# profi248/backuwup

Measured on AMD Instinct MI355X. Metric: GB/s chunked+hashed+deduped (whole node, 1/2/4/8 GPU), bit-exact vs CPU, higher is better.
Workload: dtype u8

## Files before the change

backuwup_amd/csrc/bw_blake3.hip:

```cpp
#include "bw_device.h"
#include "bw_internal.h"

namespace bw {
#if BW_CLOCK_STAMPS
__device__ ClockLog* g_clk_b3 = nullptr;
void clock_log_register_b3(void* log) { hipMemcpyToSymbol(HIP_SYMBOL(g_clk_b3), &log, sizeof(log)); }
#endif


typedef uint32_t u32x4_a4 __attribute__((ext_vector_type(4), aligned(4)));

__device__ uint32_t g_b3_dummy[36];

__device__ __forceinline__ void load_words(const uint32_t* src, uint32_t w[17]) {
    const u32x4_a4* q = (const u32x4_a4*)src;
    const u32x4_a4 a = q[0], b = q[1], c = q[2], d = q[3];
    w[0] = a.x; w[1] = a.y; w[2] = a.z; w[3] = a.w; w[4] = b.x; w[5] = b.y; w[6] = b.z; w[7] = b.w;
    w[8] = c.x; w[9] = c.y; w[10] = c.z; w[11] = c.w; w[12] = d.x; w[13] = d.y; w[14] = d.z; w[15] = d.w;
    w[16] = src[16];
}

template <bool PREFETCH>
__device__ __forceinline__ void b3_leaf(const uint8_t* __restrict__ data, uint64_t ls, uint32_t ll, uint64_t bend,
                                        uint64_t t, uint32_t root, uint32_t cv[8]) {
// ... 195 lines not shown
        switch (u + 16) { B3_CUT_CASE8(16) B3_CUT_CASE8(24) B3_CUT_CASE8(32) B3_CUT_CASE8(40) default: break; }
    }
}

__device__ __attribute__((aligned(128))) uint4 g_b3_zero_line[8];

__device__ __forceinline__ void b3_line_load(const uint4* __restrict__ src, uint32_t w[32]) {
#pragma unroll
    for (int k = 0; k < 8; k++) {
        const uint4 v = src[k];
        w[4 * k] = v.x; w[4 * k + 1] = v.y; w[4 * k + 2] = v.z; w[4 * k + 3] = v.w;
    }
}

__device__ __forceinline__ void b3_line_block(uint32_t m[16], uint32_t blk, uint32_t glen, uint32_t nblk, uint64_t n,
                                              uint64_t first, uint32_t cv[8], uint32_t (*s_leaf)[8][256], int me) {
    const uint32_t left = glen - 64 * blk;
    const uint32_t blen = glen == 0 ? 0 : (left < 64 ? left : 64);
    if (blen < 64) {
        const uint32_t whole = blen >> 2, rem = blen & 3;
        const uint32_t pmask = rem ? 0xffffffffu >> (32 - 8 * rem) : 0;
#pragma unroll
        for (uint32_t i = 0; i < 16; i++) m[i] = i < whole ? m[i] : (i == whole ? m[i] & pmask : 0);
    }
    const uint32_t bil = blk & 15, leaf = blk >> 4;
    const bool last = bil == 15 || blk + 1 == nblk;
    if (bil == 0) b3_iv(cv);
    uint32_t flags = bil == 0 ? B3_CHUNK_START : 0;
    if (last) flags |= B3_CHUNK_END | (n == 1 ? B3_ROOT : 0);
    b3_compress(cv, m, blen, first + leaf, flags);
    if (last) {
#pragma unroll
        for (int i = 0; i < 8; i++) s_leaf[leaf][i][me] = cv[i];
    }
}

constexpr uint64_t B3_SMALL_LEAVES = 64;

template <bool COH>
__device__ __forceinline__ uint32_t cv_ld(const uint32_t* p) {
    if constexpr (COH) return __hip_atomic_load(const_cast<uint32_t*>(p), __ATOMIC_RELAXED, __HIP_MEMORY_SCOPE_AGENT);
    else return *p;
}
template <bool COH>
__device__ __forceinline__ void cv_st(uint32_t* p, uint32_t v) {
    if constexpr (COH) __hip_atomic_store(p, v, __ATOMIC_RELAXED, __HIP_MEMORY_SCOPE_AGENT);
    else *p = v;
}
__device__ __forceinline__ void wave_mem_drain() { asm volatile("s_waitcnt vmcnt(0)" ::: "memory"); }

template <bool COH>
__device__ __forceinline__ void b3_small_blob(uint64_t blob, const uint64_t* ctr, const BlobArrays& b,
                                              uint32_t* __restrict__ cv_buf, uint8_t* __restrict__ digests);
template <bool COH, int NT = 64>
__device__ __forceinline__ void b3_upper_wave(uint64_t blob, uint64_t len, const BlobArrays& b, uint32_t* __restrict__ cv_buf,
                              uint32_t* __restrict__ cv_tmp, uint8_t* __restrict__ digests);

template <int MINW, bool FUSED>
__global__ __launch_bounds__(256, MINW) void k_b3_lines(const uint8_t* __restrict__ data, const uint64_t* ctr,
                                                        BlobArrays b, uint32_t* __restrict__ cv_buf,
                                                        uint32_t* __restrict__ cv_tmp, uint8_t* __restrict__ digests) {
    const uint64_t ng = ctr[C_NGROUPS];
    const uint64_t g0 = (uint64_t)blockIdx.x * blockDim.x + threadIdx.x;
    const bool live = g0 < ng;
    if (FUSED ? (ng == 0 || g0 - (threadIdx.x & 63) >= ng) : !live) return;
#if BW_CLOCK_STAMPS
    ClockStamp clk((blockIdx.x & 3) == 0 ? g_clk_b3 : nullptr, 1);
#endif
    const uint64_t g = live ? g0 : ng - 1;
    const uint64_t nb = ctr[C_NBLOBS];
    uint64_t lo = 0, hi = nb;
    while (lo < hi) {
        const uint64_t mid = (lo + hi) >> 1;
        if (b.goff[mid] <= g) lo = mid + 1;
        else hi = mid;
    }
    const uint64_t blob = lo - 1;
    BW_ASSERT(lo >= 1 && blob < b.cap);
    const uint64_t start = b.start[blob], len = b.len[blob], gi = g - b.goff[blob];
    const uint32_t gs = b.gshift, G = 1u << gs;
    BW_ASSERT(gs <= 2 && start + len <= b.data_len && (gi << gs) * B3_LEAF_BYTES <= (len ? len - 1 : 0));
    const uint64_t n = len == 0 ? 1 : (len + B3_LEAF_BYTES - 1) / B3_LEAF_BYTES;
    const uint64_t first = gi << gs;
    const uint32_t k = (uint32_t)(n - first < G ? n - first : G);
    __shared__ uint32_t s_leaf[4][8][256];
    const int me = threadIdx.x;
    const uint8_t* gp = data + start + first * B3_LEAF_BYTES;
    const uint32_t o = (uint32_t)((uintptr_t)gp & 127);
    const uint32_t q = o >> 2, sh = o & 3;
    const uint32_t uq = __builtin_amdgcn_readfirstlane(q);
    uint32_t cv[8];
    if (__builtin_amdgcn_ballot_w64(q != uq) == 0) {
        const uint64_t rest = len - first * B3_LEAF_BYTES;
        const uint32_t glen = len == 0 ? 0 : (uint32_t)(rest < G * B3_LEAF_BYTES ? rest : G * B3_LEAF_BYTES);
        const uint32_t nblk = glen == 0 ? 1 : (glen + 63) / 64;
        const uint4* lp = (const uint4*)(gp - o);
        const uint32_t nlines = glen == 0 ? 0 : (o + glen + 127) / 128;
        uint32_t a[32], c[32];
        b3_line_load(nlines > 0 ? lp : g_b3_zero_line, a);
        b3_line_load(nlines > 1 ? lp + 8 : g_b3_zero_line, c);
#pragma unroll 1
        for (uint32_t p = 0;; p += 2) {
            uint32_t m[16];
            b3_cut<0>(a, c, uq, sh, m);
            b3_line_block(m, 2 * p, glen, nblk, n, first, cv, s_leaf, me);
            if (2 * p + 1 >= nblk) break;
            b3_cut<1>(a, c, uq, sh, m);
            b3_line_load(p + 2 < nlines ? lp + 8 * (p + 2) : g_b3_zero_line, a);
            b3_line_block(m, 2 * p + 1, glen, nblk, n, first, cv, s_leaf, me);
// ... 16 lines not shown
            for (int i = 0; i < 8; i++) s_leaf[t][i][me] = cv[i];
        }
    }
    uint32_t acc[8], r[8];
#pragma unroll
    for (int i = 0; i < 8; i++) acc[i] = s_leaf[0][i][me];
    if (k >= 2) {
#pragma unroll
        for (int i = 0; i < 8; i++) r[i] = s_leaf[1][i][me];
        b3_parent(acc, r, (n == 2 || (n == 4 && false)) ? B3_ROOT : 0, acc);
    }
    if (k == 4) {
        uint32_t l2[8], l3[8];
#pragma unroll
        for (int i = 0; i < 8; i++) { l2[i] = s_leaf[2][i][me]; l3[i] = s_leaf[3][i][me]; }
        b3_parent(l2, l3, 0, r);
        b3_parent(acc, r, n == 4 ? B3_ROOT : 0, acc);
    } else if (k == 3) {
#pragma unroll
        for (int i = 0; i < 8; i++) r[i] = s_leaf[2][i][me];
        b3_parent(acc, r, n == 3 ? B3_ROOT : 0, acc);
    }
    if (n <= G) store_digest(digests + blob * 32, acc);
    else {
        uint32_t* o8 = cv_buf + g * 8;
#pragma unroll
        for (int i = 0; i < 8; i++) cv_st<FUSED>(o8 + i, acc[i]);
    }
    if constexpr (FUSED) {
        const uint32_t lane = threadIdx.x & 63;
        const bool upper = live && n > G;
        const uint64_t pb = bw_shfl_up64(blob, 1);
        const bool head = upper && (lane == 0 || pb != blob);
        const uint64_t H = __ballot(head), U = __ballot(upper);
        if (H == 0) return;
        wave_mem_drain();
        bool complete = false;
        if (head) {
            const uint64_t above = H & ~((2ull << lane) - 1);
            const uint32_t end = above ? (uint32_t)__builtin_ctzll(above) : 64u;
            const uint64_t run = (end == 64 ? ~0ull : ((1ull << end) - 1)) & ~((1ull << lane) - 1);
            const uint32_t cnt = (uint32_t)__popcll(U & run);
            const uint32_t total = (uint32_t)((n + G - 1) >> gs);
            const uint32_t old = __hip_atomic_fetch_add(b.gdone + blob, cnt, __ATOMIC_RELAXED, __HIP_MEMORY_SCOPE_AGENT);
            BW_ASSERT(old + cnt <= total);
            complete = old + cnt == total;
            if (complete) b.gdone[blob] = 0;
        }
        const uint64_t C = __ballot(complete);
        if (C == 0) return;
        for (uint64_t m = C; m; m &= m - 1) {
            const int h = __builtin_ctzll(m);
            const uint64_t cb = bw_shfl64(blob, h), cl = bw_shfl64(len, h);
            if (cl > (uint64_t)B3_SMALL_LEAVES * B3_LEAF_BYTES) b3_upper_wave<true>(cb, cl, b, cv_buf, cv_tmp, digests);
        }
        if (complete) b3_small_blob<true>(blob, ctr, b, cv_buf, digests);
    }
}


template <bool COH>
__device__ __forceinline__ void b3_small_blob(uint64_t blob, const uint64_t* ctr, const BlobArrays& b,
                                              uint32_t* __restrict__ cv_buf, uint8_t* __restrict__ digests) {
    if (blob >= ctr[C_NBLOBS]) return;
    const uint64_t len = b.len[blob];
    const uint64_t n = len == 0 ? 1 : (len + B3_LEAF_BYTES - 1) / B3_LEAF_BYTES;
    const uint32_t gs = b.gshift;
    if (n <= (1u << gs) || n > B3_SMALL_LEAVES) return;
    uint32_t* g = cv_buf + b.goff[blob] * 8;
    const uint32_t m2 = (uint32_t)(n >> gs);
    const bool tail = (n & ((1u << gs) - 1)) != 0;
    uint32_t depth = 0;
    for (uint32_t i = 0; i < m2; i++) {
        uint32_t carry[8];
#pragma unroll
        for (int w = 0; w < 8; w++) carry[w] = cv_ld<COH>(g + i * 8 + w);
        for (uint32_t c = i + 1; (c & 1) == 0; c >>= 1) {
            uint32_t l[8];
            depth--;
#pragma unroll
            for (int w = 0; w < 8; w++) l[w] = cv_ld<COH>(g + depth * 8 + w);
            b3_parent(l, carry, (!tail && i + 1 == m2 && depth == 0) ? B3_ROOT : 0, carry);
        }
#pragma unroll
        for (int w = 0; w < 8; w++) cv_st<COH>(g + depth * 8 + w, carry[w]);
        depth++;
    }
    uint32_t acc[8];
    bool have = false;
    if (tail) {
#pragma unroll
        for (int w = 0; w < 8; w++) acc[w] = cv_ld<COH>(g + m2 * 8 + w);
        have = true;
    }
    while (depth > 0) {
        depth--;
        uint32_t t[8];
#pragma unroll
        for (int w = 0; w < 8; w++) t[w] = cv_ld<COH>(g + depth * 8 + w);
        if (!have) {
#pragma unroll
            for (int w = 0; w < 8; w++) acc[w] = t[w];
            have = true;
        } else {
            b3_parent(t, acc, depth == 0 ? B3_ROOT : 0, acc);
        }
    }
    store_digest(digests + blob * 32, acc);
}

__device__ __forceinline__ void b3_shfl8(const uint32_t x[8], int src, uint32_t out[8]) {
#pragma unroll
    for (int w = 0; w < 8; w++) out[w] = __shfl(x[w], src, 64);
}

template <bool COH, int NT>
__device__ __forceinline__ void b3_upper_wave(uint64_t blob, uint64_t len, const BlobArrays& b, uint32_t* __restrict__ cv_buf,
                              uint32_t* __restrict__ cv_tmp, uint8_t* __restrict__ digests) {
    static_assert(NT == 64 || NT == 256, "a wave or a 4-wave workgroup per blob");
    const uint32_t lane = threadIdx.x & 63, t = threadIdx.x & (NT - 1);
    const uint64_t n = (len + B3_LEAF_BYTES - 1) / B3_LEAF_BYTES;
    uint32_t* src = cv_buf + b.goff[blob] * 8;
    uint32_t* dst = cv_tmp + b.goff[blob] * 8;
    const uint32_t gs = b.gshift;
    uint64_t cnt = n >> gs;
    bool have = (n & ((1u << gs) - 1)) != 0;
    uint32_t acc[8];
#pragma unroll
    for (int w = 0; w < 8; w++) acc[w] = 0;
    if (have && t == NT - 1) {
#pragma unroll
        for (int w = 0; w < 8; w++) acc[w] = cv_ld<COH>(src + cnt * 8 + w);
    }
    int l = (int)gs;
    while (cnt > 64) {
        const bool spine = cnt & 1;
        const uint64_t next = cnt / 2;
        for (uint64_t base = 0; base < next; base += NT - 1) {
            const uint64_t i = base + t;
            const bool pair = t < NT - 1 && i < next;
            const bool fold = t == NT - 1 && base == 0 && spine && have;
            if (pair || fold) {
                uint32_t L[8], R[8], P[8];
                const uint64_t li = pair ? 2 * i : cnt - 1;
#pragma unroll
                for (int w = 0; w < 8; w++) L[w] = cv_ld<COH>(src + li * 8 + w);
#pragma unroll
                for (int w = 0; w < 8; w++) R[w] = pair ? cv_ld<COH>(src + (li + 1) * 8 + w) : acc[w];
                b3_parent(L, R, 0, P);
                if (pair) {
#pragma unroll
                    for (int w = 0; w < 8; w++) cv_st<COH>(dst + i * 8 + w, P[w]);
                } else {
#pragma unroll
                    for (int w = 0; w < 8; w++) acc[w] = P[w];
                }
            }
        }
        if (spine && !have && t == NT - 1) {
#pragma unroll
            for (int w = 0; w < 8; w++) acc[w] = cv_ld<COH>(src + (cnt - 1) * 8 + w);
        }
        have |= spine;
        if constexpr (COH) wave_mem_drain();
        if constexpr (NT == 64) {
            __builtin_amdgcn_fence(__ATOMIC_RELEASE, "workgroup");
            __builtin_amdgcn_wave_barrier();
            __builtin_amdgcn_fence(__ATOMIC_ACQUIRE, "workgroup");
        } else {
            __syncthreads();
        }
        uint32_t* t = src;
        src = dst;
        dst = t;
        cnt = next;
        l++;
    }
    if (NT > 64 && t / 64 != (NT - 1) / 64) return;
    uint32_t x[8];
#pragma unroll
    for (int w = 0; w < 8; w++) x[w] = lane < cnt ? cv_ld<COH>(src + lane * 8 + w) : 0;
    for (;;) {
        const bool spine = cnt & 1;
        const uint32_t next = (uint32_t)(cnt / 2);
        uint32_t L[8], R[8], T[8], P[8];
        b3_shfl8(x, (int)(2 * lane) & 63, L);
        b3_shfl8(x, (int)(2 * lane + 1) & 63, R);
        b3_shfl8(x, (int)(cnt - 1), T);
        const bool pair = lane < next;
        const bool fold = lane == 63 && spine && have;
        if (pair || fold) {
            const uint32_t root = pair ? (n == (2ull << l) ? B3_ROOT : 0) : ((n >> (l + 1)) == 0 ? B3_ROOT : 0);
            uint32_t A[8], B[8];
#pragma unroll
            for (int w = 0; w < 8; w++) { A[w] = pair ? L[w] : T[w]; B[w] = pair ? R[w] : acc[w]; }
            b3_parent(A, B, root, P);
        }
        if (lane == 63 && spine) {
#pragma unroll
            for (int w = 0; w < 8; w++) acc[w] = have ? P[w] : T[w];
        }
        have |= spine;
        if (next == 0) break;
        if (pair) {
#pragma unroll
            for (int w = 0; w < 8; w++) x[w] = P[w];
        }
        cnt = next;
        l++;
    }
    if (lane == 63) store_digest(digests + blob * 32, acc);
}

__global__ __launch_bounds__(256) void k_b3_upper(const uint64_t* ctr, BlobArrays b, uint32_t* __restrict__ cv_buf,
                                                  uint32_t* __restrict__ cv_tmp, uint8_t* __restrict__ digests,
                                                  uint32_t small_blocks, uint32_t per_block) {
    if (blockIdx.x < small_blocks) {
        b3_small_blob<false>((uint64_t)blockIdx.x * blockDim.x + threadIdx.x, ctr, b, cv_buf, digests);
        return;
    }
    const uint64_t nblobs = ctr[C_NBLOBS];
    if (per_block) {
        const uint64_t one_group = (uint64_t)B3_LEAF_BYTES << b.gshift;
        for (uint64_t blob = blockIdx.x - small_blocks; blob < nblobs; blob += gridDim.x - small_blocks) {
            const uint64_t len = b.len[blob];
            if (len <= one_group) continue;
            b3_upper_wave<false, 256>(blob, len, b, cv_buf, cv_tmp, digests);
        }
        return;
    }
    const uint64_t waves = (uint64_t)(gridDim.x - small_blocks) * (blockDim.x / 64);
    for (uint64_t blob = (uint64_t)(blockIdx.x - small_blocks) * (blockDim.x / 64) + threadIdx.x / 64; blob < nblobs;
         blob += waves) {
        const uint64_t len = b.len[blob];
        if (len <= (uint64_t)B3_SMALL_LEAVES * B3_LEAF_BYTES) continue;
        b3_upper_wave<false, 64>(blob, len, b, cv_buf, cv_tmp, digests);
    }
}

#ifndef BW_B3_LINES_MINW
#define BW_B3_LINES_MINW 3
#endif
#ifndef B3_UPPER_BLOCK_BLOBS
#define B3_UPPER_BLOCK_BLOBS 8192
#endif

__global__ __launch_bounds__(256, BW_B3_LINES_MINW) void k_b3_calib(uint32_t blocks_per_lane, uint32_t* sink,
                                                                    uint64_t* stamps) {
    uint32_t cv[8], m[16];
    b3_iv(cv);
#pragma unroll
    for (int i = 0; i < 16; i++) m[i] = threadIdx.x * 16 + i + blockIdx.x;
    uint64_t t0 = 0, r0 = 0;
    if (threadIdx.x == 0) {
        t0 = __builtin_amdgcn_s_memtime();
        r0 = __builtin_amdgcn_s_memrealtime();
    }
    for (uint32_t k = 0; k < blocks_per_lane; k++) {
        m[0] ^= k;
        b3_compress(cv, m, 64, k, 0);
    }
    if (threadIdx.x == 0) {
        stamps[2 * blockIdx.x] = __builtin_amdgcn_s_memtime() - t0;
        stamps[2 * blockIdx.x + 1] = __builtin_amdgcn_s_memrealtime() - r0;
    }
    if (cv[0] == 0x9e3779b9u && cv[1] == 0x7f4a7c15u) sink[0] = cv[2];
}

void launch_b3_calib(hipStream_t st, uint32_t n_blocks, uint32_t blocks_per_lane, uint32_t* sink, uint64_t* stamps) {
    hipLaunchKernelGGL(k_b3_calib, dim3(n_blocks), dim3(256), 0, st, blocks_per_lane, sink, stamps);
}

uint32_t b3_calib_blocks_per_cu() { return BW_B3_LINES_MINW; }

void launch_blake3(hipStream_t st, const uint8_t* data, const uint64_t* ctr, BlobArrays b, uint64_t max_blobs,
                   uint64_t max_groups, uint32_t* cv_buf, uint32_t* cv_tmp, uint8_t* digests, int max_leaves,
                   hipEvent_t between, int loads, hipStream_t upper, hipEvent_t leaf_done, hipEvent_t mark) {
    if (!max_blobs) {
        if (leaf_done) hipEventRecord(leaf_done, st);
        return;
    }
#ifndef BW_B3_DYN_LDS
#define BW_B3_DYN_LDS 0
#endif
#if BW_DIAG
    const bool fused = loads == B3_LOADS_LINES && b.gdone;
    if (fused)
        hipLaunchKernelGGL((k_b3_lines<BW_B3_LINES_MINW, true>), dim3((unsigned)((max_groups + 255) / 256)), dim3(256), 0, st,
                           data, ctr, b, cv_buf, cv_tmp, digests);
    else if (loads == B3_LOADS_PAIRS)
        hipLaunchKernelGGL((k_b3_groups<false, 1, true>), dim3((unsigned)((max_groups + 255) / 256)), dim3(256), BW_B3_DYN_LDS, st,
                           data, ctr, b, cv_buf, digests);
    else if (loads == B3_LOADS_PREFETCH)
        hipLaunchKernelGGL((k_b3_groups<true, 1, false>), dim3((unsigned)((max_groups + 255) / 256)), dim3(256), 0, st,
                           data, ctr, b, cv_buf, digests);
    else
#else
    const bool fused = false;
    (void)loads;
#endif
        hipLaunchKernelGGL((k_b3_lines<BW_B3_LINES_MINW, false>), dim3((unsigned)((max_groups + 255) / 256)), dim3(256), 0, st,
                           data, ctr, b, cv_buf, cv_tmp, digests);
    if (leaf_done) hipEventRecord(leaf_done, st);
    if (mark) hipEventRecord(mark, st);
    if (between) hipEventRecord(between, st);
    if (upper != st) hipStreamWaitEvent(upper, between, 0);
    st = upper;
    if (max_leaves > (1 << b.gshift) && !fused) {
        const bool per_block = max_blobs <= B3_UPPER_BLOCK_BLOBS;
        const uint64_t small = per_block ? 0 : (max_blobs + 255) / 256;
        uint64_t big = per_block ? max_blobs : (max_leaves > (int)B3_SMALL_LEAVES ? (max_blobs + 3) / 4 : 0);
        if (big > 4096) big = 4096;
        hipLaunchKernelGGL(k_b3_upper, dim3((unsigned)(small + big)), dim3(256), 0, st, ctr, b, cv_buf, cv_tmp, digests,
                           (uint32_t)small, (uint32_t)per_block);
    }
}

}
```

backuwup_amd/csrc/bw_capi.hip:

```cpp
#include <math.h>
#include <stdio.h>
#include <stdlib.h>
#include <string.h>

#include <algorithm>
#include <atomic>
#include <chrono>
#include <functional>
#include <mutex>
#include <string>
#include <thread>
#include <unordered_map>
#include <vector>

#include "../../include/backuwup_gpu.h"
#include "bw_device.h"
#include "bw_internal.h"
#include "bw_tables.inc"

using namespace bw;

static const uint64_t H_MASKS[26] = BW_MASKS_INIT;

#include "bw_ctx.h"
// ... 450 lines not shown
            return BW_OK;
        case BW_OPT_SPLIT:
            if (v < 1 || v > 2) return BW_EINVAL;
            c->split = (int)v;
            return BW_OK;
        case BW_OPT_SCAN_SMALL_BYTES:
            c->scan_small_bytes = v;
            return c->helper ? bw_set_option(c->helper, opt, v) : BW_OK;
        case BW_OPT_ORDER_HASH:
            if (v > 1) return BW_EINVAL;
            c->order_hash = v != 0;
            return BW_OK;
        case BW_OPT_CAND_CAP:
            c->cand_cap_forced = v;
            return c->helper ? bw_set_option(c->helper, opt, v) : BW_OK;
        case BW_OPT_SCAN_WAVES:
            if (v != 8 && v != 16) return BW_EINVAL;
            c->scan_waves = (int)v;
            return c->helper ? bw_set_option(c->helper, opt, v) : BW_OK;
        case BW_OPT_LATENCY_STREAM:
            if (v && !c->hi) {
                hipSetDevice(c->device);
                int least = 0, greatest = 0;
                HIPCHK(c, hipDeviceGetStreamPriorityRange(&least, &greatest));
                HIPCHK(c, hipStreamCreateWithPriority(&c->hi, hipStreamNonBlocking, greatest));
                for (hipEvent_t* e : {&c->e_scan, &c->e_lat, &c->e_b3, &c->e_end})
                    HIPCHK(c, hipEventCreateWithFlags(e, EV_ORDER));
            }
            c->lat_split = v != 0;
            return BW_OK;
        case BW_OPT_ZSTD_SLOTS:
            if (v < 1 || v > (1u << 20)) return BW_EINVAL;
            hipSetDevice(c->device);
            hipStreamSynchronize(c->stream);
            zstd_work_limits(c->zw, v, 0);
            return BW_OK;
        case BW_OPT_ZSTD_BATCH_BYTES:
            if (v < (1u << 20)) return BW_EINVAL;
            zstd_work_limits(c->zw, 0, v);
            return BW_OK;
        case BW_OPT_B3_LOADS:
            if (v > B3_LOADS_LINES) return BW_EINVAL;
            c->b3_loads = (int)v;
            return c->helper ? bw_set_option(c->helper, opt, v) : BW_OK;
        case BW_OPT_PROFILE_MASK:
            if (__builtin_popcountll(v) < 2 || v >= (2u << BW_N_STAGES)) return BW_EINVAL;
            c->prof_mask = (uint32_t)v;
            return c->helper ? bw_set_option(c->helper, opt, v) : BW_OK;
        case BW_OPT_B3_GROUP:
            if (v != 0 && v != 1 && v != 2 && v != 4) return BW_EINVAL;
            c->b3_group = (int)v;
            return c->helper ? bw_set_option(c->helper, opt, v) : BW_OK;
        case BW_OPT_B3_UPPER:
            if (v > 1) return BW_EINVAL;
            c->b3_fused = v == 1;
            return c->helper ? bw_set_option(c->helper, opt, v) : BW_OK;
        case BW_OPT_SCAN_FIRST:
            if (v > 2) return BW_EINVAL;
            c->scan_first = (int)v;
            return c->helper ? bw_set_option(c->helper, opt, v) : BW_OK;
        case BW_OPT_STAGE_CHUNK:
            if (v < 4096) return BW_EINVAL;
            hipSetDevice(c->device);
            if (c->copy) hipStreamSynchronize(c->copy);
            for (int r = 0; r < STAGE_RING; r++) free_host(c->ring[r]);
            c->stage_chunk = v;
            return BW_OK;
        default: return BW_EINVAL;
    }
}


extern "C" int bw_index_create(int device, bw_index** out) {
    if (!out) return BW_EINVAL;
    *out = nullptr;
    bw_index* x = new bw_index();
    if (int rc = index_init(x, device)) {
        index_release(x);
        return rc;
    }
    *out = x;
    return BW_OK;
}

extern "C" void bw_index_destroy(bw_index* x) { index_release(x); }

extern "C" int bw_attach_index(bw_ctx* c, bw_index* x) {
    if (!c) return BW_EINVAL;
    if (!x) x = c->own_idx;
    if (x->device != c->device) {
        c->err = "index and context live on different devices";
        return BW_EINVAL;
    }
    if (x == c->idx) return BW_OK;
    hipSetDevice(c->device);
    HIPCHK(c, hipStreamSynchronize(c->stream));
    bw_index* old = c->idx;
    if (x != c->own_idx) x->refs++;
    c->idx = x;
    c->idx_mark = 0;
    if (old != c->own_idx) index_release(old);
    if (c->helper) return bw_attach_index(c->helper, x);
    return BW_OK;
}

extern "C" int bw_index_reset(bw_ctx* c, uint64_t hint) {
    if (!c) return BW_EINVAL;
    hipSetDevice(c->device);
// ... 329 lines not shown
        if (int r6 = enqueue_scan()) return r6;
    uint64_t* ctr = slot_ctr(s);
    hipStream_t st = c->stream;

    BlobArrays b{P<uint64_t>(c->b_start), P<uint64_t>(c->b_len), P<uint64_t>(c->b_goff), P<uint32_t>(c->b_file),
                 P<uint32_t>(c->b_kind), P<uint64_t>(c->b_fend), P<uint64_t>(c->b_ghash), max_blobs, data_len,
                 c->b3_fused ? P<uint32_t>(c->b_gdone) : nullptr, gshift};

    const bool split = c->lat_split;
    hipStream_t lat = split ? c->hi : st;
    if (split) {
        HIPCHK(c, hipEventRecord(c->e_scan, st));
        HIPCHK(c, hipStreamWaitEvent(lat, c->e_scan, 0));
    }
    prof_mark(c, BW_STAGE_COMPACT, lat);
    if (ncf)
        launch_compact(lat, d_data, data_len, n_tiles, mk, P<uint32_t>(c->tile_count), P<uint64_t>(c->tile_slots),
                       P<uint64_t>(c->tile_off), P<uint64_t>(c->cand), cand_cap, P<uint32_t>(c->ovf), ctr,
                       P<uint64_t>(c->tile_btot));
    prof_mark(c, BW_STAGE_RESOLVE, lat);
    if (ncf) {
        launch_chains(lat, d_data, data_len, mk, P<uint64_t>(c->cand), P<uint64_t>(c->tile_off), ctr, d_segs,
                      nseg, P<uint64_t>(c->chains), P<uint32_t>(c->chain_n), P<uint64_t>(c->chain_cptr),
                      P<uint64_t>(c->merge), force_serial);
        launch_resolve(lat, d_data, data_len, mk, P<uint64_t>(c->cand), P<uint64_t>(c->tile_off), ctr,
                       d_segs, nseg, d_cfs, ncf, P<uint64_t>(c->chains),
                       P<uint32_t>(c->chain_n), P<uint64_t>(c->merge), P<uint64_t>(c->seg_M), P<uint32_t>(c->seg_cnt),
                       P<uint32_t>(c->cf_invalid), P<uint64_t>(c->fb_starts), P<uint64_t>(c->fb_count), force_serial);
    }
    prof_mark(c, BW_STAGE_ASSEMBLE, lat);
    launch_assemble(lat, ctr, d_units, nunits, d_segs, d_cfs,
                    P<uint64_t>(c->chains), P<uint32_t>(c->chain_n), P<uint64_t>(c->seg_M), P<uint32_t>(c->cf_invalid),
                    P<uint64_t>(c->fb_starts), P<uint64_t>(c->fb_count), b, P<uint64_t>(c->ucnt),
                    P<uint64_t>(c->ubtot));
    if (ncf) launch_cut_hash(lat, d_data, mk, ctr, b, max_blobs);
    else HIPCHK(c, hipMemsetAsync(c->b_ghash.p, 0, max_blobs * 8, lat));
    if (split) {
        HIPCHK(c, hipEventRecord(c->e_lat, lat));
        HIPCHK(c, hipStreamWaitEvent(st, c->e_lat, 0));
    }

    prof_mark(c, BW_STAGE_B3LEAF, st);
    if (do_hash) {
        hipEvent_t mark = c->prof && ((c->prof_mask >> BW_STAGE_B3TREE) & 1) ? c->ev[c->ev_set][BW_STAGE_B3TREE] : nullptr;
        hipEvent_t between = split ? c->e_b3 : nullptr;
        bw_index* x = c->idx;
        std::unique_lock<std::mutex> lk(x->mu, std::defer_lock);
        const bool order = c->order_hash || order_force;
        if (order) {
            lk.lock();
            if (x->hash_tail_set) HIPCHK(c, hipStreamWaitEvent(st, x->hash_tail, 0));
        }
        launch_blake3(st, d_data, ctr, b, max_blobs, max_groups, P<uint32_t>(c->cv), P<uint32_t>(c->cv2),
                      P<uint8_t>(s.digests), max_leaves, between, c->b3_loads, lat, order ? x->hash_tail : nullptr, mark);
        if (order) x->hash_tail_set = true;
    } else {
        prof_mark(c, BW_STAGE_B3TREE, st);
        if (split) {
            HIPCHK(c, hipEventRecord(c->e_b3, st));
            HIPCHK(c, hipStreamWaitEvent(lat, c->e_b3, 0));
        }
        HIPCHK(c, hipMemsetAsync(s.digests.p, 0, max_blobs * 32, lat));
    }
    if (d_data == P<uint8_t>(s.input)) HIPCHK(c, hipEventRecord(s.input_free, st));
    phase(3);
    prof_mark(c, BW_STAGE_DEDUP, lat);
    uint64_t want = 0;
    bool zero_copy = false;
    if (stage)
        if (int r5 = stage_prepare(c, s, max_blobs, &want, &zero_copy)) return r5;
    auto pack = [&](hipStream_t ps) {
        prof_mark(c, BW_STAGE_PACK, ps);
        launch_pack(ps, ctr, b, d_fstart, P<uint8_t>(s.digests), do_dedup ? P<uint8_t>(s.is_dup) : nullptr,
                    slot_records(s), max_blobs, do_dedup ? P<uint64_t>(c->idx->dstate) : nullptr,
                    zero_copy ? (uint8_t*)s.res.p : nullptr, want);
    };
    if (do_dedup) {
        if (int r4 = dedup_device(c, P<uint8_t>(s.digests), ctr + C_DEDUPN, 0, max_blobs, P<uint8_t>(s.is_dup), lat,
                                  pack))
            return r4;
        s.mark = c->idx_mark;
    } else {
        pack(lat);
    }
    phase(4);
    if (split) {
        prof_mark(c, BW_N_STAGES, lat);
        HIPCHK(c, hipEventRecord(c->e_end, lat));
        HIPCHK(c, hipStreamWaitEvent(st, c->e_end, 0));
    }
    if (!split) prof_mark(c, BW_N_STAGES);
    if (c->prof) c->ev_pending[c->ev_set] = true;
    HIPCHK(c, hipGetLastError());
    s.max_blobs = max_blobs;
    s.geo_tiles = n_tiles;
    s.geo_cfiles = ncf;
    s.geo_segs = nseg;
    s.geo_tile_bytes = tile_bytes;
    s.geo_seg_bytes = L;
    s.dedup = do_dedup;
    s.hashed = do_hash;
    s.comm = nullptr;
    s.ex_state = 0;
    s.ex_rc = 0;
    s.ex_first = 0;
    s.ex_n = ~0ull;
    if (stage)
        if (int r5 = stage_results(c, s, zero_copy, want)) return r5;
    phase(5);
    c->host_batches += c->host_timing;
    return BW_OK;
}

static Slot& claim_slot(bw_ctx* c, uint64_t* ticket) {
    const uint64_t t = c->next_ticket++;
    Slot& s = c->slots[(t - 1) % (uint64_t)c->depth];
    if (s.ex_state == 1 && s.comm) exchange_progress(s.comm, &s);
    if (s.ex_state == 2) hipStreamWaitEvent(c->stream, s.done, 0);
    s.ticket = t;
    c->last_ticket = t;
    if (ticket) *ticket = t;
    return s;
}

static const bw_params* params_or_default(const bw_params* prm, bw_params* def) {
    if (prm) return prm;
    bw_params_default(def);
    return def;
}

static int ensure_helper(bw_ctx* c) {
    if (c->helper) return BW_OK;
    bw_ctx* h = nullptr;
    if (int rc = bw_create(c->device, &h)) return rc;
    h->is_helper = true;
    h->depth = c->depth;
    h->scan_small_bytes = c->scan_small_bytes;
    h->cand_cap_forced = c->cand_cap_forced;
    h->b3_loads = c->b3_loads;
    h->scan_waves = c->scan_waves;
    h->b3_group = c->b3_group;
    h->b3_fused = c->b3_fused;
    h->prof_mask = c->prof_mask;
    h->scan_first = c->scan_first;
    if (c->lat_split && bw_set_option(h, BW_OPT_LATENCY_STREAM, 1) != BW_OK) {
        bw_destroy(h);
        return BW_EHIP;
    }
    if (int rc = bw_attach_index(h, c->idx)) {
        bw_destroy(h);
        return rc;
    }
    if (c->prof) bw_profile_enable(h, 1);
    if (!c->e_split) HIPCHK(c, hipEventCreateWithFlags(&c->e_split, EV_ORDER));
    if (!c->e_tail) HIPCHK(c, hipEventCreateWithFlags(&c->e_tail, EV_ORDER));
    c->helper = h;
    return BW_OK;
}

static uint64_t split_point(bw_ctx* c, uint64_t data_len, const uint64_t* flen, uint64_t nf, const bw_params* prm) {
    if (c->split < 2 || c->is_helper || nf < 2 || (prm->flags & (BW_F_NO_DEDUP | BW_F_NO_HASH))) return 0;
    if (data_len > c->split_max) return 0;
    uint64_t total = 0;
    for (uint64_t f = 0; f < nf; f++) total += flen[f];
    if (total < c->split_min) return 0;
    uint64_t acc = 0;
    for (uint64_t f = 0; f + 1 < nf; f++) {
        acc += flen[f];
        if (2 * acc >= total) return f + 1;
    }
    return nf - 1;
}

static int submit_split(bw_ctx* c, Slot& s, const uint8_t* d_data, uint64_t data_len, const uint64_t* foff,
                        const uint64_t* flen, uint64_t nf, const bw_params* prm) {
    s.tail_ticket = 0;
    Masks mk;
    if (int rc = validate_batch(c, data_len, foff, flen, nf, prm, &mk)) return rc;
    const uint64_t f0 = split_point(c, data_len, flen, nf, prm);
    if (!f0) return submit(c, s, d_data, data_len, foff, flen, nf, prm);
    if (int rc = ensure_helper(c)) return rc;
    bw_ctx* h = c->helper;
    HIPCHK(c, hipEventRecord(c->e_split, c->stream));
    if (int rc = submit(c, s, d_data, data_len, foff, flen, f0, prm, true, true)) return rc;
    HIPCHK(c, hipStreamWaitEvent(h->stream, c->e_split, 0));
    uint64_t t2 = 0;
    Slot& s2 = claim_slot(h, &t2);
    if (int rc = submit(h, s2, d_data, data_len, foff + f0, flen + f0, nf - f0, prm, true, true)) {
        s2.ticket = 0;
        c->err = "tail part: " + h->err;
        return rc;
    }
    HIPCHK(c, hipEventRecord(c->e_tail, h->stream));
    HIPCHK(c, hipStreamWaitEvent(c->stream, c->e_tail, 0));
    if (d_data == P<uint8_t>(s.input)) HIPCHK(c, hipEventRecord(s.input_free, c->stream));
// ... 737 lines not shown
```

backuwup_amd/csrc/bw_ctx.h:

```cpp
#pragma once
#include <atomic>
#include <functional>
#include <mutex>
#include <string>
#include <thread>
#include <vector>

#include "../../include/backuwup_gpu.h"
#include "bw_internal.h"

using namespace bw;

namespace bwx {

struct DevBuf {
    void* p = nullptr;
    size_t cap = 0;
};

struct PinBuf {
    void* p = nullptr;
    size_t cap = 0;
};

// ... 32 lines not shown

using namespace bwx;

struct bw_index {
    int device = 0;
    std::mutex mu;
    std::atomic<int> refs{1};
    DevBuf table, log, dstate;
    uint64_t table_cap = 0, log_cap = 0;
    uint64_t log_hi = 0;
    uint64_t enq_total = 0;
    hipEvent_t tail = nullptr;
    bool tail_set = false;
    hipStream_t tail_stream = nullptr;
    hipEvent_t hash_tail = nullptr, scan_tail = nullptr;
    bool hash_tail_set = false, scan_tail_set = false;
};

struct bw_ctx {
    int device = 0;
    hipStream_t own = nullptr, stream = nullptr, copy = nullptr;
    std::string err;

    DevBuf tile_count, tile_slots, tile_off, tile_btot, cand, ovf;
    DevBuf meta, chains, chain_n, chain_cptr, merge, seg_M, seg_cnt, cf_invalid, fb_starts, fb_count;
    DevBuf b_start, b_len, b_goff, b_file, b_kind, b_fend, b_ghash;
    DevBuf b_gdone;
    DevBuf cv, cv2, data, scratch, ucnt, ubtot;
    DevBuf bk_blk, bk_pack, bk_v;
    DevBuf ex_rbk, ex_v, ex_rv;
    hipStream_t ex_st = nullptr;

    Slot slots[MAX_DEPTH];
    int depth = 2;
    uint64_t next_ticket = 1, last_ticket = 0;
    uint64_t last_n = 0;
    int split = 1;
    uint64_t split_min = 64ull << 20, split_max = 4ull << 30;
    bw_ctx* helper = nullptr;
    bool is_helper = false;
    hipEvent_t e_split = nullptr, e_tail = nullptr;
    Slot sync_slot;

    PinBuf ring[STAGE_RING];
    hipEvent_t ring_ev[STAGE_RING] = {};
    bool ring_set[STAGE_RING] = {};
    uint64_t stage_chunk = 64ull << 20;

    uint64_t scan_small_bytes = SCAN_SMALL_BYTES;
    bool order_hash = false;
    uint64_t cand_cap_forced = 0;
    int b3_group = 0;
    bool b3_fused = false;
    int b3_loads = B3_LOADS_LINES;
    int scan_waves = 16;
    bool lat_split = false;
    hipStream_t hi = nullptr;
    hipEvent_t e_scan = nullptr, e_lat = nullptr, e_b3 = nullptr, e_end = nullptr;
    uint64_t cand_override = 0;

    DevBuf seal_items, seal_keys, seal_parts, seal_ok, seal_io;
    PinBuf seal_stage;
    hipEvent_t seal_done = nullptr;
    bool seal_pending = false;

    DevBuf pk_blobs, pk_files, pk_hdr, pk_src, pk_out, ix_io, ix_tab, ix_dig;
    std::vector<PackBlob> h_pk_blobs;
    std::vector<PackFileDesc> h_pk_files;
    hipEvent_t pk_done = nullptr;
    bool pk_pending = false;

    PinBuf msg_stage;

    ZstdWork* zw = nullptr;
    struct ZsLane {
        hipStream_t st = nullptr;
        hipStream_t own_st = nullptr;
        hipEvent_t ready = nullptr;
        ZstdWork* w = nullptr;
        std::thread th;
        uint64_t ticket = 0;
        std::vector<uint64_t> so, sl, dof, fl;
        int rc = 0;
        std::string err;
    };
    ZsLane zs_lanes[BW_ZSTD_LANES];
    uint64_t zs_next = 1;
    DevBuf zs_io;
    DevBuf pk_stage;
    std::vector<uint64_t> pk_stage_off, pk_stage_len;

    bw_index* own_idx = nullptr;
    bw_index* idx = nullptr;
    uint64_t idx_mark = 0;

    bool host_timing = false;
    double host_ms[6] = {};
    uint64_t host_batches = 0;

    bool prof = false;
    uint32_t prof_mask = (2u << BW_N_STAGES) - 1;
    int scan_first = 2;
    hipEvent_t ev[2][BW_N_STAGES + 1] = {};
    bool ev_pending[2] = {false, false};
    int ev_set = 0;
    double stage_ms[BW_N_STAGES] = {};
// ... 35 lines not shown
```

backuwup_amd/csrc/bw_internal.h:

```cpp
#pragma once
#include <algorithm>
#include <string>
#include <thread>
#include <vector>
#include <hip/hip_runtime.h>
#include <stdint.h>

#include "../../include/backuwup_gpu.h"

#ifndef BW_DIAG
#define BW_DIAG 0
#endif

namespace bw {

constexpr int SCAN_BLOCK = 1024;
#ifndef BW_SCAN_STRIP
#define BW_SCAN_STRIP 2048
#endif
#ifndef BW_SCAN_CAP
#define BW_SCAN_CAP 16
#endif
constexpr int SCAN_STRIP = BW_SCAN_STRIP;
constexpr uint64_t SCAN_TILE = 64ull * SCAN_STRIP;
// ... 55 lines not shown
    uint32_t seg;
    uint32_t cfile;
};

struct BlobArrays {
    uint64_t* start;
    uint64_t* len;
    uint64_t* goff;
    uint32_t* file;
    uint32_t* kind;
    uint64_t* fend;
    uint64_t* ghash;
    uint64_t cap;
    uint64_t data_len;
    uint32_t* gdone = nullptr;
    uint32_t gshift = 2;
};

bool launch_scan(hipStream_t st, const uint8_t* data, uint64_t n_bytes, uint64_t n_tiles,
                 const Masks& mk, uint32_t* tile_count, uint64_t* tile_slots, uint32_t* ovf_list,
                 uint64_t* ctr, int waves );
void launch_compact(hipStream_t st, const uint8_t* data, uint64_t n_bytes, uint64_t n_tiles,
                    const Masks& mk, uint32_t* tile_count, uint64_t* tile_slots,
                    uint64_t* tile_off, uint64_t* cand, uint64_t cand_cap, uint32_t* ovf_list,
                    uint64_t* ctr, uint64_t* scratch );
void launch_chains(hipStream_t st, const uint8_t* data, uint64_t data_len, const Masks& mk, const uint64_t* cand,
                   const uint64_t* tile_off, uint64_t* ctr, const SegDesc* segs, uint64_t nseg,
                   uint64_t* chains, uint32_t* chain_n, uint64_t* chain_cptr, uint64_t* merge,
                   int force_serial);
void launch_resolve(hipStream_t st, const uint8_t* data, uint64_t data_len, const Masks& mk, const uint64_t* cand,
                    const uint64_t* tile_off, uint64_t* ctr, const SegDesc* segs, uint64_t nseg,
                    const CFileDesc* cfiles, uint64_t ncf, const uint64_t* chains,
                    const uint32_t* chain_n, const uint64_t* merge, uint64_t* seg_M,
                    uint32_t* seg_cnt, uint32_t* cf_invalid, uint64_t* fb_starts,
                    uint64_t* fb_count, int force_serial);
void launch_assemble(hipStream_t st, uint64_t* ctr, const UnitDesc* units, uint64_t nunits,
                     const SegDesc* segs, const CFileDesc* cfiles, const uint64_t* chains,
                     const uint32_t* chain_n, const uint64_t* seg_M, const uint32_t* cf_invalid,
                     const uint64_t* fb_starts, const uint64_t* fb_count, BlobArrays b,
                     uint64_t* ucnt , uint64_t* ubtot );
void launch_upload(hipStream_t st, const void* host_src, void* dst, uint64_t bytes);
void launch_zero(hipStream_t st, uint64_t* p, uint32_t n);
void launch_cut_hash(hipStream_t st, const uint8_t* data, const Masks& mk, const uint64_t* ctr,
                     BlobArrays b, uint64_t max_blobs);


enum { B3_LOADS_PREFETCH = 0, B3_LOADS_PAIRS = 1, B3_LOADS_LINES = 2 };
void launch_blake3(hipStream_t st, const uint8_t* data, const uint64_t* ctr, BlobArrays b,
                   uint64_t max_blobs, uint64_t max_groups, uint32_t* cv_buf,
                   uint32_t* cv_tmp , uint8_t* digests, int max_leaves,
                   hipEvent_t between , int loads,
                   hipStream_t upper ,
                   hipEvent_t leaf_done = nullptr ,
                   hipEvent_t mark = nullptr );
void launch_b3_calib(hipStream_t st, uint32_t n_blocks, uint32_t blocks_per_lane, uint32_t* sink, uint64_t* stamps);
uint32_t b3_calib_blocks_per_cu();
enum DState : int { D_LOGLEN = 0, D_NUNIQUE = 1, D_LOST = 2, D_BUCKET_OVF = 3, D_DONE = 4, D_COUNT = 5 };
void launch_table_clear(hipStream_t st, uint64_t* table, uint64_t cap);
void launch_dedup(hipStream_t st, uint64_t* table, uint64_t cap, uint8_t* log, uint64_t* dstate,
                  const uint8_t* digests, const uint64_t* n_dev, uint64_t n_host, uint64_t max_n,
                  uint8_t* is_dup);
void launch_rehash(hipStream_t st, uint64_t* table, uint64_t cap, const uint8_t* log,
                   const uint64_t* dstate, uint64_t max_n);
void launch_partition(hipStream_t st, const uint8_t* digests, uint64_t n, uint32_t n_owners,
                      uint8_t* out, uint64_t* perm, uint64_t* counts_dev);
void launch_scatter(hipStream_t st, const uint8_t* verdict, const uint64_t* perm, uint64_t n,
                    uint8_t* is_dup);
void launch_bucket_partition(hipStream_t st, const uint8_t* digests, const uint64_t* n_dev, uint64_t max_n,
                             uint32_t n_owners, uint64_t cap, uint8_t* out, uint64_t* perm, uint64_t* counts,
                             uint64_t* blk, uint64_t* err);
void launch_bucket_gather(hipStream_t st, const uint8_t* buckets, const uint64_t* counts, uint32_t n_src, uint64_t cap,
                          uint8_t* out, uint64_t* n_out);
void launch_bucket_expand(hipStream_t st, const uint64_t* counts, uint32_t n_src, uint64_t cap, const uint8_t* v_in,
                          uint8_t* v_out);
void launch_bucket_scatter(hipStream_t st, const uint8_t* verdict, const uint64_t* perm, const uint64_t* counts,
                           uint32_t n_owners, uint64_t cap, uint8_t* is_dup, uint8_t* packed = nullptr);
void launch_pack(hipStream_t st, uint64_t* ctr, BlobArrays b, const uint64_t* file_start,
                 const uint8_t* digests, const uint8_t* is_dup, uint8_t* out, uint64_t max_blobs,
                 const uint64_t* dstate, uint8_t* host = nullptr, uint64_t host_n = 0);
void launch_index_snapshot(hipStream_t st, const uint64_t* dstate, uint64_t* ctr);
void launch_owner_partition(hipStream_t st, const uint8_t* digests, const uint64_t* n_dev, uint64_t max_n,
                            uint32_t n_owners, uint8_t* out, uint64_t* perm, uint64_t* msg, uint64_t* blk);
void launch_copy_u64(hipStream_t st, const uint64_t* src, uint64_t* dst, uint32_t n);
void launch_owner_scatter(hipStream_t st, const uint8_t* verdict, const uint64_t* perm, uint64_t n, uint8_t* is_dup,
                          uint8_t* packed);

constexpr uint32_t PIECE_BLOCKS = 8192;
constexpr int SEAL_THREADS = 1024;

struct SealItem {
    uint64_t src_off, len, dst_off, piece0;
    uint32_t nonce[3];
    uint32_t info_len;
    uint8_t info[56];
    uint32_t raw_len, wd;
};

struct SealKey {
    uint32_t rk[60];
    uint32_t H[4], E0[4], HP[4], H64[4];
    uint32_t P[6][4];
    uint32_t R1[4];
};

struct SealPads {
    uint32_t istate[8], ostate[8];
};
// ... 77 lines not shown
```

Baseline: 1942.

## Process multiple upper BLAKE3 trees per wave using sub-wave teams

The upper-tree BLAKE3 kernel now assigns a team of 32 lanes (configurable to 16 or 64) per blob instead of a full wave, so each wave reduces several blobs' chaining-value trees at once. Shuffles are made team-relative, and loops use wave-wide ballots so teams with different depths stay converged. Non-coherent CV loads and stores are also vectorised to 16-byte accesses. This aims to cut idle lanes when most blobs have few groups, at the cost of more divergence and extra iterations for teams with shallow trees.

```diff
diff --git a/backuwup_amd/csrc/bw_blake3.hip b/backuwup_amd/csrc/bw_blake3.hip
--- a/backuwup_amd/csrc/bw_blake3.hip
+++ b/backuwup_amd/csrc/bw_blake3.hip
@@ -271,9 +271,30 @@
 template <bool COH>
 __device__ __forceinline__ void b3_small_blob(uint64_t blob, const uint64_t* ctr, const BlobArrays& b,
                                               uint32_t* __restrict__ cv_buf, uint8_t* __restrict__ digests);
+template <bool COH>
+__device__ __forceinline__ void cv_ld8(const uint32_t* p, uint32_t out[8]) {
+    if constexpr (COH) {
+#pragma unroll
+        for (int w = 0; w < 8; w++) out[w] = cv_ld<true>(p + w);
+    } else {
+        const uint4 a = ((const uint4*)p)[0], c = ((const uint4*)p)[1];
+        out[0] = a.x; out[1] = a.y; out[2] = a.z; out[3] = a.w; out[4] = c.x; out[5] = c.y; out[6] = c.z; out[7] = c.w;
+    }
+}
+template <bool COH>
+__device__ __forceinline__ void cv_st8(uint32_t* p, const uint32_t v[8]) {
+    if constexpr (COH) {
+#pragma unroll
+        for (int w = 0; w < 8; w++) cv_st<true>(p + w, v[w]);
+    } else {
+        ((uint4*)p)[0] = make_uint4(v[0], v[1], v[2], v[3]);
+        ((uint4*)p)[1] = make_uint4(v[4], v[5], v[6], v[7]);
+    }
+}
+
 template <bool COH, int NT = 64>
-__device__ __forceinline__ void b3_upper_wave(uint64_t blob, uint64_t len, const BlobArrays& b, uint32_t* __restrict__ cv_buf,
-                              uint32_t* __restrict__ cv_tmp, uint8_t* __restrict__ digests);
+__device__ __forceinline__ void b3_upper_wave(uint64_t blob, uint64_t len, bool live, const BlobArrays& b,
+                              uint32_t* __restrict__ cv_buf, uint32_t* __restrict__ cv_tmp, uint8_t* __restrict__ digests);
 
 template <int MINW, bool FUSED>
 __global__ __launch_bounds__(256, MINW) void k_b3_lines(const uint8_t* __restrict__ data, const uint64_t* ctr,
@@ -396,7 +417,7 @@
         for (uint64_t m = C; m; m &= m - 1) {
             const int h = __builtin_ctzll(m);
             const uint64_t cb = bw_shfl64(blob, h), cl = bw_shfl64(len, h);
-            if (cl > (uint64_t)B3_SMALL_LEAVES * B3_LEAF_BYTES) b3_upper_wave<true>(cb, cl, b, cv_buf, cv_tmp, digests);
+            if (cl > (uint64_t)B3_SMALL_LEAVES * B3_LEAF_BYTES) b3_upper_wave<true>(cb, cl, true, b, cv_buf, cv_tmp, digests);
         }
         if (complete) b3_small_blob<true>(blob, ctr, b, cv_buf, digests);
     }
@@ -458,81 +479,91 @@
     for (int w = 0; w < 8; w++) out[w] = __shfl(x[w], src, 64);
 }
 
+template <int NT>
+__device__ __forceinline__ bool b3_any(bool p) {
+    if constexpr (NT < 64) return __builtin_amdgcn_ballot_w64(p) != 0;
+    else return p;
+}
+
 template <bool COH, int NT>
-__device__ __forceinline__ void b3_upper_wave(uint64_t blob, uint64_t len, const BlobArrays& b, uint32_t* __restrict__ cv_buf,
-                              uint32_t* __restrict__ cv_tmp, uint8_t* __restrict__ digests) {
-    static_assert(NT == 64 || NT == 256, "a wave or a 4-wave workgroup per blob");
+__device__ __forceinline__ void b3_upper_wave(uint64_t blob, uint64_t len, bool live, const BlobArrays& b,
+                              uint32_t* __restrict__ cv_buf, uint32_t* __restrict__ cv_tmp, uint8_t* __restrict__ digests) {
+    static_assert(NT == 16 || NT == 32 || NT == 64 || NT == 256, "a team, a wave or a 4-wave workgroup per blob");
+    constexpr uint32_t RL = NT < 64 ? NT : 64;
     const uint32_t lane = threadIdx.x & 63, t = threadIdx.x & (NT - 1);
+    const uint32_t rl = lane & (RL - 1), tb = lane & ~(RL - 1);
     const uint64_t n = (len + B3_LEAF_BYTES - 1) / B3_LEAF_BYTES;
-    uint32_t* src = cv_buf + b.goff[blob] * 8;
-    uint32_t* dst = cv_tmp + b.goff[blob] * 8;
+    const uint64_t goff = live ? b.goff[blob] : 0;
+    uint32_t* src = cv_buf + goff * 8;
+    uint32_t* dst = cv_tmp + goff * 8;
     const uint32_t gs = b.gshift;
-    uint64_t cnt = n >> gs;
-    bool have = (n & ((1u << gs) - 1)) != 0;
+    uint64_t cnt = live ? n >> gs : 0;
+    bool have = live && (n & ((1u << gs) - 1)) != 0;
     uint32_t acc[8];
 #pragma unroll
     for (int w = 0; w < 8; w++) acc[w] = 0;
-    if (have && t == NT - 1) {
-#pragma unroll
-        for (int w = 0; w < 8; w++) acc[w] = cv_ld<COH>(src + cnt * 8 + w);
-    }
+    if (have && t == NT - 1) cv_ld8<COH>(src + cnt * 8, acc);
     int l = (int)gs;
-    while (cnt > 64) {
-        const bool spine = cnt & 1;
+    while (b3_any<NT>(cnt > RL)) {
+        const bool act = cnt > RL;
+        const bool spine = act && (cnt & 1);
         const uint64_t next = cnt / 2;
-        for (uint64_t base = 0; base < next; base += NT - 1) {
+        for (uint64_t base = 0; b3_any<NT>(act && base < next); base += NT - 1) {
             const uint64_t i = base + t;
-            const bool pair = t < NT - 1 && i < next;
+            const bool pair = act && t < NT - 1 && i < next;
             const bool fold = t == NT - 1 && base == 0 && spine && have;
             if (pair || fold) {
                 uint32_t L[8], R[8], P[8];
                 const uint64_t li = pair ? 2 * i : cnt - 1;
-#pragma unroll
-                for (int w = 0; w < 8; w++) L[w] = cv_ld<COH>(src + li * 8 + w);
-#pragma unroll
-                for (int w = 0; w < 8; w++) R[w] = pair ? cv_ld<COH>(src + (li + 1) * 8 + w) : acc[w];
+                cv_ld8<COH>(src + li * 8, L);
+                if (pair) {
+                    cv_ld8<COH>(src + (li + 1) * 8, R);
+                } else {
+#pragma unroll
+                    for (int w = 0; w < 8; w++) R[w] = acc[w];
+                }
                 b3_parent(L, R, 0, P);
                 if (pair) {
-#pragma unroll
-                    for (int w = 0; w < 8; w++) cv_st<COH>(dst + i * 8 + w, P[w]);
+                    cv_st8<COH>(dst + i * 8, P);
                 } else {
 #pragma unroll
                     for (int w = 0; w < 8; w++) acc[w] = P[w];
                 }
             }
         }
-        if (spine && !have && t == NT - 1) {
-#pragma unroll
-            for (int w = 0; w < 8; w++) acc[w] = cv_ld<COH>(src + (cnt - 1) * 8 + w);
-        }
+        if (spine && !have && t == NT - 1) cv_ld8<COH>(src + (cnt - 1) * 8, acc);
         have |= spine;
         if constexpr (COH) wave_mem_drain();
-        if constexpr (NT == 64) {
+        if constexpr (NT <= 64) {
             __builtin_amdgcn_fence(__ATOMIC_RELEASE, "workgroup");
             __builtin_amdgcn_wave_barrier();
             __builtin_amdgcn_fence(__ATOMIC_ACQUIRE, "workgroup");
         } else {
             __syncthreads();
         }
-        uint32_t* t = src;
-        src = dst;
-        dst = t;
-        cnt = next;
-        l++;
+        if (act) {
+            uint32_t* s = src;
+            src = dst;
+            dst = s;
+            cnt = next;
+            l++;
+        }
     }
     if (NT > 64 && t / 64 != (NT - 1) / 64) return;
     uint32_t x[8];
 #pragma unroll
-    for (int w = 0; w < 8; w++) x[w] = lane < cnt ? cv_ld<COH>(src + lane * 8 + w) : 0;
+    for (int w = 0; w < 8; w++) x[w] = 0;
+    if (rl < cnt) cv_ld8<COH>(src + rl * 8, x);
+    bool on = live;
     for (;;) {
-        const bool spine = cnt & 1;
+        const bool spine = on && (cnt & 1);
         const uint32_t next = (uint32_t)(cnt / 2);
         uint32_t L[8], R[8], T[8], P[8];
-        b3_shfl8(x, (int)(2 * lane) & 63, L);
-        b3_shfl8(x, (int)(2 * lane + 1) & 63, R);
-        b3_shfl8(x, (int)(cnt - 1), T);
-        const bool pair = lane < next;
-        const bool fold = lane == 63 && spine && have;
+        b3_shfl8(x, (int)(tb | ((2 * rl) & (RL - 1))), L);
+        b3_shfl8(x, (int)(tb | ((2 * rl + 1) & (RL - 1))), R);
+        b3_shfl8(x, (int)(tb | ((uint32_t)(cnt - 1) & (RL - 1))), T);
+        const bool pair = on && rl < next;
+        const bool fold = rl == RL - 1 && spine && have;
         if (pair || fold) {
             const uint32_t root = pair ? (n == (2ull << l) ? B3_ROOT : 0) : ((n >> (l + 1)) == 0 ? B3_ROOT : 0);
             uint32_t A[8], B[8];
@@ -540,46 +571,72 @@
             for (int w = 0; w < 8; w++) { A[w] = pair ? L[w] : T[w]; B[w] = pair ? R[w] : acc[w]; }
             b3_parent(A, B, root, P);
         }
-        if (lane == 63 && spine) {
+        if (rl == RL - 1 && spine) {
 #pragma unroll
             for (int w = 0; w < 8; w++) acc[w] = have ? P[w] : T[w];
         }
         have |= spine;
-        if (next == 0) break;
+        if (next == 0) on = false;
+        if (!b3_any<NT>(on)) break;
         if (pair) {
 #pragma unroll
             for (int w = 0; w < 8; w++) x[w] = P[w];
         }
-        cnt = next;
-        l++;
-    }
-    if (lane == 63) store_digest(digests + blob * 32, acc);
+        if (on) {
+            cnt = next;
+            l++;
+        }
+    }
+    if (live && rl == RL - 1) store_digest(digests + blob * 32, acc);
+}
+
+#ifndef B3_UPPER_TEAM
+#define B3_UPPER_TEAM 32
+#endif
+
+template <int NT>
+__device__ __forceinline__ void b3_upper_many(const uint64_t* ctr, const BlobArrays& b, uint32_t* __restrict__ cv_buf,
+                                              uint32_t* __restrict__ cv_tmp, uint8_t* __restrict__ digests,
+                                              uint32_t small_blocks) {
+    constexpr uint32_t PER_WAVE = 64 / NT;
+    const uint64_t nblobs = ctr[C_NBLOBS];
+    const uint64_t waves = (uint64_t)(gridDim.x - small_blocks) * (blockDim.x / 64);
+    const uint64_t wave = (uint64_t)(blockIdx.x - small_blocks) * (blockDim.x / 64) + threadIdx.x / 64;
+    for (uint64_t first = wave * PER_WAVE; first < nblobs; first += waves * PER_WAVE) {
+        const uint64_t blob = first + (threadIdx.x & 63) / NT;
+        const uint64_t len = blob < nblobs ? b.len[blob] : 0;
+        const bool live = len > (uint64_t)B3_SMALL_LEAVES * B3_LEAF_BYTES;
+        if (!b3_any<NT>(live)) continue;
+        b3_upper_wave<false, NT>(blob, len, live, b, cv_buf, cv_tmp, digests);
+    }
 }
 
 __global__ __launch_bounds__(256) void k_b3_upper(const uint64_t* ctr, BlobArrays b, uint32_t* __restrict__ cv_buf,
                                                   uint32_t* __restrict__ cv_tmp, uint8_t* __restrict__ digests,
-                                                  uint32_t small_blocks, uint32_t per_block) {
+                                                  uint32_t small_blocks, uint32_t lanes) {
     if (blockIdx.x < small_blocks) {
         b3_small_blob<false>((uint64_t)blockIdx.x * blockDim.x + threadIdx.x, ctr, b, cv_buf, digests);
         return;
     }
-    const uint64_t nblobs = ctr[C_NBLOBS];
-    if (per_block) {
+    if (lanes == 256) {
+        const uint64_t nblobs = ctr[C_NBLOBS];
         const uint64_t one_group = (uint64_t)B3_LEAF_BYTES << b.gshift;
         for (uint64_t blob = blockIdx.x - small_blocks; blob < nblobs; blob += gridDim.x - small_blocks) {
             const uint64_t len = b.len[blob];
             if (len <= one_group) continue;
-            b3_upper_wave<false, 256>(blob, len, b, cv_buf, cv_tmp, digests);
+            b3_upper_wave<false, 256>(blob, len, true, b, cv_buf, cv_tmp, digests);
         }
         return;
     }
-    const uint64_t waves = (uint64_t)(gridDim.x - small_blocks) * (blockDim.x / 64);
-    for (uint64_t blob = (uint64_t)(blockIdx.x - small_blocks) * (blockDim.x / 64) + threadIdx.x / 64; blob < nblobs;
-         blob += waves) {
-        const uint64_t len = b.len[blob];
-        if (len <= (uint64_t)B3_SMALL_LEAVES * B3_LEAF_BYTES) continue;
-        b3_upper_wave<false, 64>(blob, len, b, cv_buf, cv_tmp, digests);
-    }
+#if BW_DIAG
+    if (lanes != B3_UPPER_TEAM) {
+        if (lanes == 64) b3_upper_many<64>(ctr, b, cv_buf, cv_tmp, digests, small_blocks);
+        else if (lanes == 32) b3_upper_many<32>(ctr, b, cv_buf, cv_tmp, digests, small_blocks);
+        else b3_upper_many<16>(ctr, b, cv_buf, cv_tmp, digests, small_blocks);
+        return;
+    }
+#endif
+    b3_upper_many<B3_UPPER_TEAM>(ctr, b, cv_buf, cv_tmp, digests, small_blocks);
 }
 
 #ifndef BW_B3_LINES_MINW
@@ -619,7 +676,8 @@
 
 void launch_blake3(hipStream_t st, const uint8_t* data, const uint64_t* ctr, BlobArrays b, uint64_t max_blobs,
                    uint64_t max_groups, uint32_t* cv_buf, uint32_t* cv_tmp, uint8_t* digests, int max_leaves,
-                   hipEvent_t between, int loads, hipStream_t upper, hipEvent_t leaf_done, hipEvent_t mark) {
+                   hipEvent_t between, int loads, hipStream_t upper, hipEvent_t leaf_done, hipEvent_t mark,
+                   int upper_team) {
     if (!max_blobs) {
         if (leaf_done) hipEventRecord(leaf_done, st);
         return;
@@ -652,12 +710,14 @@
     st = upper;
     if (max_leaves > (1 << b.gshift) && !fused) {
         const bool per_block = max_blobs <= B3_UPPER_BLOCK_BLOBS;
+        const uint32_t lanes = per_block ? 256 : (BW_DIAG && upper_team ? (uint32_t)upper_team : B3_UPPER_TEAM);
+        const uint64_t per = 256 / lanes;
         const uint64_t small = per_block ? 0 : (max_blobs + 255) / 256;
-        uint64_t big = per_block ? max_blobs : (max_leaves > (int)B3_SMALL_LEAVES ? (max_blobs + 3) / 4 : 0);
+        uint64_t big = per_block || max_leaves > (int)B3_SMALL_LEAVES ? (max_blobs + per - 1) / per : 0;
         if (big > 4096) big = 4096;
         hipLaunchKernelGGL(k_b3_upper, dim3((unsigned)(small + big)), dim3(256), 0, st, ctr, b, cv_buf, cv_tmp, digests,
-                           (uint32_t)small, (uint32_t)per_block);
-    }
-}
-
-}
+                           (uint32_t)small, lanes);
+    }
+}
+
+}
diff --git a/backuwup_amd/csrc/bw_capi.hip b/backuwup_amd/csrc/bw_capi.hip
--- a/backuwup_amd/csrc/bw_capi.hip
+++ b/backuwup_amd/csrc/bw_capi.hip
@@ -526,8 +526,9 @@
             c->b3_group = (int)v;
             return c->helper ? bw_set_option(c->helper, opt, v) : BW_OK;
         case BW_OPT_B3_UPPER:
-            if (v > 1) return BW_EINVAL;
+            if (v > 3) return BW_EINVAL;
             c->b3_fused = v == 1;
+            c->b3_team = v == 2 ? 64 : v == 3 ? 16 : 0;
             return c->helper ? bw_set_option(c->helper, opt, v) : BW_OK;
         case BW_OPT_SCAN_FIRST:
             if (v > 2) return BW_EINVAL;
@@ -963,7 +964,8 @@
             if (x->hash_tail_set) HIPCHK(c, hipStreamWaitEvent(st, x->hash_tail, 0));
         }
         launch_blake3(st, d_data, ctr, b, max_blobs, max_groups, P<uint32_t>(c->cv), P<uint32_t>(c->cv2),
-                      P<uint8_t>(s.digests), max_leaves, between, c->b3_loads, lat, order ? x->hash_tail : nullptr, mark);
+                      P<uint8_t>(s.digests), max_leaves, between, c->b3_loads, lat, order ? x->hash_tail : nullptr, mark,
+                      c->b3_team);
         if (order) x->hash_tail_set = true;
     } else {
         prof_mark(c, BW_STAGE_B3TREE, st);
@@ -1052,6 +1054,7 @@
     h->scan_waves = c->scan_waves;
     h->b3_group = c->b3_group;
     h->b3_fused = c->b3_fused;
+    h->b3_team = c->b3_team;
     h->prof_mask = c->prof_mask;
     h->scan_first = c->scan_first;
     if (c->lat_split && bw_set_option(h, BW_OPT_LATENCY_STREAM, 1) != BW_OK) {
diff --git a/backuwup_amd/csrc/bw_ctx.h b/backuwup_amd/csrc/bw_ctx.h
--- a/backuwup_amd/csrc/bw_ctx.h
+++ b/backuwup_amd/csrc/bw_ctx.h
@@ -108,6 +108,7 @@
     uint64_t cand_cap_forced = 0;
     int b3_group = 0;
     bool b3_fused = false;
+    int b3_team = 0;
     int b3_loads = B3_LOADS_LINES;
     int scan_waves = 16;
     bool lat_split = false;
diff --git a/backuwup_amd/csrc/bw_internal.h b/backuwup_amd/csrc/bw_internal.h
--- a/backuwup_amd/csrc/bw_internal.h
+++ b/backuwup_amd/csrc/bw_internal.h
@@ -131,7 +131,8 @@
                    hipEvent_t between , int loads,
                    hipStream_t upper ,
                    hipEvent_t leaf_done = nullptr ,
-                   hipEvent_t mark = nullptr );
+                   hipEvent_t mark = nullptr ,
+                   int upper_team = 0 );
 void launch_b3_calib(hipStream_t st, uint32_t n_blocks, uint32_t blocks_per_lane, uint32_t* sink, uint64_t* stamps);
 uint32_t b3_calib_blocks_per_cu();
 enum DState : int { D_LOGLEN = 0, D_NUNIQUE = 1, D_LOST = 2, D_BUCKET_OVF = 3, D_DONE = 4, D_COUNT = 5 };
```

After: 1951, median of 6. Within noise of the previous version (+0.4%).
